# praveer13/zest

Hardware: AMD Instinct MI355X
Metric: aggregate pull GB/s + P2P ratio, Llama-3.1-70B at 1/2/4/8 MI355X peers (higher is better)
Workload: dtype bf16

## Files before the change

csrc/gpu/compress.hip:

```cpp
#include <hip/hip_runtime.h>

#include <cstdint>
#include <cstdlib>

#include "zgpu.h"

namespace {

constexpr int kWave = 64;
constexpr int kWavesPerBlock = 4;
constexpr int kTabLog = 12;
constexpr uint32_t kTab = 1u << kTabLog;

__device__ __forceinline__ uint32_t lane_id() { return threadIdx.x & (kWave - 1); }

__device__ __forceinline__ uint32_t load_u32(const uint8_t* p) {
  const uintptr_t a = reinterpret_cast<uintptr_t>(p);
  const uint32_t k = uint32_t(a & 3);
  const uint32_t* w = reinterpret_cast<const uint32_t*>(a & ~uintptr_t(3));
  const uint32_t w0 = w[0];
  return k == 0 ? w0 : __builtin_amdgcn_alignbyte(w[1], w0, k);
}

__device__ __forceinline__ uint32_t put_len(uint8_t* o, uint32_t op, uint32_t r, uint32_t lane) {
  const uint32_t nff = r / 255;
  for (uint32_t i = lane; i < nff; i += kWave) o[op + i] = 0xFF;
  if (lane == 0) o[op + nff] = uint8_t(r - 255 * nff);
  return op + nff + 1;
}

__device__ __forceinline__ uint32_t emit(uint8_t* o, uint32_t op, const uint8_t* in, uint32_t lit0, uint32_t L,
                                         uint32_t off, uint32_t ml, uint32_t lane) {
  const uint32_t M = ml ? ml - 4 : 0;
  if (lane == 0) o[op] = uint8_t(((L < 15 ? L : 15) << 4) | (ml ? (M < 15 ? M : 15) : 0));
  ++op;
  if (L >= 15) op = put_len(o, op, L - 15, lane);
  for (uint32_t i = lane; i < L; i += kWave) o[op + i] = in[lit0 + i];
  op += L;
  if (ml) {
    if (lane == 0) {
      o[op] = uint8_t(off & 0xFF);
      o[op + 1] = uint8_t(off >> 8);
    }
    op += 2;
    if (M >= 15) op = put_len(o, op, M - 15, lane);
  }
  return op;
}

__global__ void __launch_bounds__(256) k_bg4_split(const uint8_t* __restrict__ data, const uint64_t* __restrict__ offs,
                                                   const uint32_t* __restrict__ lens, int n, uint8_t* __restrict__ out,
                                                   uint64_t slot) {
  const int c = __builtin_amdgcn_readfirstlane(int(blockIdx.x * kWavesPerBlock + (threadIdx.x >> 6)));
  if (c >= n) return;
  const uint32_t lane = lane_id(), len = lens[c];
  const uint8_t* s = data + offs[c];
  uint8_t* d = out + uint64_t(c) * slot;
  const uint32_t q = len >> 2, r = len & 3;
  const uint32_t g1 = q + (r > 0), g2 = g1 + q + (r > 1), g3 = g2 + q + (r > 2);
  for (uint32_t i = lane; i < len; i += kWave) {
    const uint32_t g = i & 3, j = i >> 2;
    const uint32_t base = g == 0 ? 0u : g == 1 ? g1 : g == 2 ? g2 : g3;
    d[base + j] = s[i];
  }
}

__global__ void __launch_bounds__(256) k_lz4_compress_v1(const uint8_t* __restrict__ data, const uint64_t* __restrict__ offs,
                                                      const uint32_t* __restrict__ lens, int n, uint64_t in_slot,
                                                      uint8_t* __restrict__ out, uint64_t out_slot,
                                                      uint32_t* __restrict__ out_len, uint32_t hc64, uint32_t hc256) {
  __shared__ unsigned long long tabs[kWavesPerBlock][kTab];
  const int wave = __builtin_amdgcn_readfirstlane(int(threadIdx.x >> 6));
  const int c = __builtin_amdgcn_readfirstlane(int(blockIdx.x * kWavesPerBlock + wave));
  if (c >= n) return;
  const uint32_t lane = lane_id();
  unsigned long long* tab = tabs[wave];
  for (uint32_t i = lane; i < kTab; i += kWave) tab[i] = 0;
  __builtin_amdgcn_wave_barrier();
  const uint32_t len = lens[c];
  const uint8_t* in = in_slot ? data + uint64_t(c) * in_slot : data + offs[c];
  uint8_t* o = out + uint64_t(c) * out_slot;
  uint32_t op = 11, ip = 0, anchor = 0;
  const uint32_t mend = len > 5 ? len - 5 : 0;
  while (ip + 12 <= len) {
    const uint32_t p = ip + lane;
    const bool ok = p + 12 <= len;
    const uint32_t v = ok ? load_u32(in + p) : 0;
    const uint32_t h = (v * 2654435761u) >> (32 - kTabLog);
    const unsigned long long e = ok ? tab[h] : 0ull;
    uint32_t cand = uint32_t(e >> 32) - 1;
    bool hit = ok && e != 0 && uint32_t(e) == v && cand < p && p - cand <= 65535u;
    uint32_t near = 0;
    for (int d = 32; d >= 1; --d) {
      const uint32_t u = __shfl_up(v, d, kWave);
      if (lane >= uint32_t(d) && u == v) near = d;
    }
    if (ok && near) {
      cand = p - near;
      hit = true;
    }
    const unsigned long long mask = __ballot(hit);
    const uint32_t passed = mask ? uint32_t(__builtin_ctzll(mask)) + 1 : uint32_t(kWave);
    __builtin_amdgcn_wave_barrier();
    if (ok && lane < passed) atomicMax(&tab[h], (static_cast<unsigned long long>(p + 1) << 32) | v);
    if (!mask) {
      ip += kWave;
      continue;
    }
    const int j = __builtin_ctzll(mask);
    uint32_t mp = ip + uint32_t(j);
    uint32_t mc = uint32_t(__builtin_amdgcn_readlane(int(cand), j));
    while (true) {
      const uint32_t room = (mp - anchor) < mc ? (mp - anchor) : mc;
      if (room == 0) break;
      const uint32_t k = lane + 1;
      const bool eq = k <= room && in[mp - k] == in[mc - k];
      const unsigned long long ne = __ballot(!eq);
      const uint32_t b = ne ? uint32_t(__builtin_ctzll(ne)) : uint32_t(kWave);
      mp -= b;
      mc -= b;
      if (b < uint32_t(kWave)) break;
    }
    const uint32_t maxlen = mend - mp;
    uint32_t ml = 4 + (ip + uint32_t(j) - mp);
    while (ml < maxlen) {
      const uint32_t k = ml + lane;
      const bool eq = k < maxlen && in[mc + k] == in[mp + k];
      const unsigned long long ne = __ballot(!eq);
      if (ne) {
        ml += uint32_t(__builtin_ctzll(ne));
        break;
      }
      ml += kWave;
    }
    if (ml > maxlen) ml = maxlen;
    op = emit(o, op, in, anchor, mp - anchor, mp - mc, ml, lane);
    ip = mp + ml;
    anchor = ip;
  }
  op = emit(o, op, in, anchor, len - anchor, 0, 0, lane);
  const uint32_t total = op + 4;
  if (total >= len) {
    if (lane == 0) out_len[c] = 0;
    return;
  }
  if (lane == 0) {
    const uint32_t bs = op - 11;
    const bool small = len <= 65536;
    const uint8_t hdr[11] = {0x04, 0x22, 0x4D, 0x18, 0x60, uint8_t(small ? 0x40 : 0x50),
                             uint8_t(small ? hc64 : hc256), uint8_t(bs), uint8_t(bs >> 8), uint8_t(bs >> 16),
                             uint8_t(bs >> 24)};
    for (int i = 0; i < 11; ++i) o[i] = hdr[i];
    for (int i = 0; i < 4; ++i) o[op + i] = 0;
    out_len[c] = total;
  }
}

constexpr uint32_t kTagBits = 14;
constexpr uint32_t kTagMask = (1u << kTagBits) - 1;
constexpr uint32_t kRing = 4096;
constexpr uint32_t kRingMask = kRing - 1;
constexpr uint32_t kFlush = 2048;
constexpr uint32_t kHdr = 11;

struct Staged {
  uint8_t* ring;
  uint8_t* g;
  uint32_t flushed;
};

__device__ __forceinline__ void ring_write(Staged& o, uint32_t end, uint32_t lane) {
  __builtin_amdgcn_wave_barrier();
  for (uint32_t pos = o.flushed + lane; pos < end; pos += kWave)
    if (pos >= kHdr) o.g[pos] = o.ring[pos & kRingMask];
  __builtin_amdgcn_wave_barrier();
}

__device__ __forceinline__ void maybe_flush(Staged& o, uint32_t op, uint32_t lane) {
  while (op - o.flushed >= kFlush) {
    ring_write(o, o.flushed + kFlush, lane);
    o.flushed += kFlush;
  }
}

__device__ __forceinline__ uint32_t put_len_s(Staged& o, uint32_t op, uint32_t r, uint32_t lane) {
  const uint32_t nff = r / 255;
  for (uint32_t i = lane; i < nff; i += kWave) o.ring[(op + i) & kRingMask] = 0xFF;
  if (lane == 0) o.ring[(op + nff) & kRingMask] = uint8_t(r - 255 * nff);
  return op + nff + 1;
}

__device__ __forceinline__ uint32_t emit_s(Staged& o, uint32_t op, const uint8_t* in, uint32_t lit0, uint32_t L,
                                           uint32_t off, uint32_t ml, uint32_t lane) {
  const uint32_t M = ml ? ml - 4 : 0;
  maybe_flush(o, op, lane);
  if (lane == 0) o.ring[op & kRingMask] = uint8_t(((L < 15 ? L : 15) << 4) | (ml ? (M < 15 ? M : 15) : 0));
  ++op;
  if (L >= 15) op = put_len_s(o, op, L - 15, lane);
  for (uint32_t b = 0; b < L; b += 1024) {
    maybe_flush(o, op + b, lane);
    const uint32_t n = L - b < 1024 ? L - b : 1024;
    for (uint32_t i = lane; i < n; i += kWave) o.ring[(op + b + i) & kRingMask] = in[lit0 + b + i];
  }
  op += L;
  if (ml) {
    maybe_flush(o, op, lane);
    if (lane == 0) {
      o.ring[op & kRingMask] = uint8_t(off & 0xFF);
      o.ring[(op + 1) & kRingMask] = uint8_t(off >> 8);
    }
    op += 2;
    if (M >= 15) op = put_len_s(o, op, M - 15, lane);
  }
  return op;
}

__global__ void __launch_bounds__(256) k_lz4_compress(const uint8_t* __restrict__ data, const uint64_t* __restrict__ offs,
                                                      const uint32_t* __restrict__ lens, int n, uint64_t in_slot,
                                                      uint8_t* __restrict__ out, uint64_t out_slot,
                                                      uint32_t* __restrict__ out_len, uint32_t hc64, uint32_t hc256) {
  __shared__ uint32_t tabs[kWavesPerBlock][kTab];
  __shared__ uint8_t rings[kWavesPerBlock][kRing];
  const int wave = __builtin_amdgcn_readfirstlane(int(threadIdx.x >> 6));
  const int c = __builtin_amdgcn_readfirstlane(int(blockIdx.x * kWavesPerBlock + wave));
  if (c >= n) return;
  const uint32_t lane = lane_id();
  uint32_t* tab = tabs[wave];
  for (uint32_t i = lane; i < kTab; i += kWave) tab[i] = 0;
  __builtin_amdgcn_wave_barrier();
  const uint32_t len = lens[c];
  const uint8_t* in = in_slot ? data + uint64_t(c) * in_slot : data + offs[c];
  Staged o{rings[wave], out + uint64_t(c) * out_slot, 0};
  uint32_t op = kHdr, ip = 0, anchor = 0;
  const uint32_t mend = len > 5 ? len - 5 : 0;
  while (ip + 12 <= len) {
    const uint32_t p = ip + lane;
    const bool ok = p + 12 <= len;
    const uint32_t v = ok ? load_u32(in + p) : 0;
    const uint32_t hv = v * 2654435761u;
    const uint32_t h = hv >> (32 - kTabLog);
    const uint32_t tag = hv & kTagMask;
    const uint32_t e = ok ? tab[h] : 0u;
    uint32_t cand = (e >> kTagBits) - 1;
    bool hit = ok && e != 0 && (e & kTagMask) == tag && cand < p && p - cand <= 65535u;
    if (hit) hit = load_u32(in + cand) == v;
    uint32_t near = 0;
    for (int d = 32; d >= 1; --d) {
      const uint32_t u = __shfl_up(v, d, kWave);
      if (lane >= uint32_t(d) && u == v) near = d;
    }
    if (ok && near) {
      cand = p - near;
      hit = true;
    }
    const unsigned long long mask = __ballot(hit);
    const uint32_t passed = mask ? uint32_t(__builtin_ctzll(mask)) + 1 : uint32_t(kWave);
    __builtin_amdgcn_wave_barrier();
    if (ok && lane < passed) atomicMax(&tab[h], ((p + 1) << kTagBits) | tag);
    if (!mask) {
      ip += kWave;
      continue;
    }
    const int j = __builtin_ctzll(mask);
    uint32_t mp = ip + uint32_t(j);
    uint32_t mc = uint32_t(__builtin_amdgcn_readlane(int(cand), j));
    while (true) {
      const uint32_t room = (mp - anchor) < mc ? (mp - anchor) : mc;
      if (room == 0) break;
      const uint32_t k = lane + 1;
      const bool eq = k <= room && in[mp - k] == in[mc - k];
      const unsigned long long ne = __ballot(!eq);
      const uint32_t b = ne ? uint32_t(__builtin_ctzll(ne)) : uint32_t(kWave);
      mp -= b;
      mc -= b;
      if (b < uint32_t(kWave)) break;
    }
    const uint32_t maxlen = mend - mp;
    uint32_t ml = 4 + (ip + uint32_t(j) - mp);
    while (ml < maxlen) {
      const uint32_t k = ml + lane;
      const bool eq = k < maxlen && in[mc + k] == in[mp + k];
      const unsigned long long ne = __ballot(!eq);
      if (ne) {
        ml += uint32_t(__builtin_ctzll(ne));
        break;
      }
      ml += kWave;
    }
    if (ml > maxlen) ml = maxlen;
    op = emit_s(o, op, in, anchor, mp - anchor, mp - mc, ml, lane);
    ip = mp + ml;
    anchor = ip;
  }
  op = emit_s(o, op, in, anchor, len - anchor, 0, 0, lane);
  const uint32_t total = op + 4;
  if (total >= len) {
    if (lane == 0) out_len[c] = 0;
    return;
  }
  maybe_flush(o, op, lane);
  if (lane < 4) o.ring[(op + lane) & kRingMask] = 0;
  ring_write(o, total, lane);
  if (lane == 0) {
    const uint32_t bs = op - kHdr;
    const bool small = len <= 65536;
    const uint8_t hdr[kHdr] = {0x04, 0x22, 0x4D, 0x18, 0x60, uint8_t(small ? 0x40 : 0x50),
                               uint8_t(small ? hc64 : hc256), uint8_t(bs), uint8_t(bs >> 8), uint8_t(bs >> 16),
                               uint8_t(bs >> 24)};
    for (uint32_t i = 0; i < kHdr; ++i) o.g[i] = hdr[i];
    out_len[c] = total;
  }
}

bool compress_v1() {
  const char* e = getenv("ZG_COMPRESS");
  return e && e[0] == 'v' && e[1] == '1';
}

__global__ void __launch_bounds__(256) k_pack_frames(const uint64_t* __restrict__ src, const uint32_t* __restrict__ clen,
                                                     const uint32_t* __restrict__ ulen, const uint8_t* __restrict__ scheme,
                                                     const uint64_t* __restrict__ out_off, int n, uint8_t* __restrict__ out) {
  const int c = __builtin_amdgcn_readfirstlane(int(blockIdx.x * kWavesPerBlock + (threadIdx.x >> 6)));
  if (c >= n) return;
  const uint32_t lane = lane_id(), cl = clen[c], ul = ulen[c];
  uint8_t* d = out + out_off[c];
  if (lane < 8) {
    const uint32_t b = lane == 0 ? 0u : lane < 4 ? (cl >> (8 * (lane - 1))) & 0xFF
                                  : lane == 4 ? scheme[c] : (ul >> (8 * (lane - 5))) & 0xFF;
    d[lane] = uint8_t(b);
  }
  const uint8_t* s = reinterpret_cast<const uint8_t*>(src[c]);
  for (uint32_t i = lane; i < cl; i += kWave) d[8 + i] = s[i];
}

}

extern "C" {

hipError_t zg_compress_chunks(const uint8_t* data, const uint64_t* offs, const uint32_t* lens, int n, int bg4,
                              uint8_t* scratch, uint64_t in_slot, uint8_t* out, uint64_t out_slot, uint32_t* out_len,
                              uint32_t hc64, uint32_t hc256, hipStream_t stream) {
  if (n <= 0) return hipSuccess;
  const dim3 grid((n + kWavesPerBlock - 1) / kWavesPerBlock);
  auto* kern = compress_v1() ? k_lz4_compress_v1 : k_lz4_compress;
  if (bg4) {
    hipLaunchKernelGGL(k_bg4_split, grid, dim3(256), 0, stream, data, offs, lens, n, scratch, in_slot);
    hipLaunchKernelGGL(kern, grid, dim3(256), 0, stream, scratch, offs, lens, n, in_slot, out, out_slot, out_len,
                       hc64, hc256);
  } else {
    hipLaunchKernelGGL(kern, grid, dim3(256), 0, stream, data, offs, lens, n, uint64_t(0), out, out_slot, out_len,
                       hc64, hc256);
  }
  return hipGetLastError();
}

hipError_t zg_pack_frames(const uint64_t* src, const uint32_t* clen, const uint32_t* ulen, const uint8_t* scheme,
                          const uint64_t* out_off, int n, uint8_t* out, hipStream_t stream) {
  if (n <= 0) return hipSuccess;
  hipLaunchKernelGGL(k_pack_frames, dim3((n + kWavesPerBlock - 1) / kWavesPerBlock), dim3(256), 0, stream, src, clen,
                     ulen, scheme, out_off, n, out);
  return hipGetLastError();
}

}
```

Before: 62.46.

## Stage LZ4 input in a register window read via ds_bpermute

The compressor keeps a sliding window of input in wave registers (four rows of 256 bytes plus a prefetch row) and reads hash words, candidate verification bytes, short match extensions and literals through ds_bpermute instead of scattered global byte loads. Candidate checking becomes a loop that compares a 64-byte span around each hit, which gives the backward and forward extension for free inside that span. It is meant to cut global memory latency in the match-finding loop. In exchange it adds many bpermute operations per step, more registers per lane, and a more complex control flow, which may lower occupancy.

```diff
diff --git a/csrc/gpu/compress.hip b/csrc/gpu/compress.hip
--- a/csrc/gpu/compress.hip
+++ b/csrc/gpu/compress.hip
@@ -190,17 +190,112 @@
   return op + nff + 1;
 }
 
-__device__ __forceinline__ uint32_t emit_s(Staged& o, uint32_t op, const uint8_t* in, uint32_t lit0, uint32_t L,
-                                           uint32_t off, uint32_t ml, uint32_t lane) {
+constexpr uint32_t kRow = 4 * kWave;
+constexpr uint32_t kWinRows = 4;
+constexpr uint32_t kWin = kRow * kWinRows;
+constexpr uint32_t kSpanBack = 16;
+constexpr uint32_t kSpanFwd = kWave - kSpanBack - 4;
+
+struct Window {
+  uint32_t w0, w1, w2, w3, nxt;
+  const uint32_t* base;
+  uint32_t a0, endq;
+  int32_t wq;
+};
+
+__device__ __forceinline__ uint32_t win_load_row(const Window& W, int32_t q0, uint32_t lane) {
+  const uint32_t q = uint32_t(q0) + 4 * lane;
+  return q < W.endq ? W.base[q >> 2] : 0u;
+}
+
+__device__ __forceinline__ void win_load_all(Window& W, int32_t wq, uint32_t lane) {
+  W.wq = wq;
+  W.w0 = win_load_row(W, wq, lane);
+  W.w1 = win_load_row(W, wq + int32_t(kRow), lane);
+  W.w2 = win_load_row(W, wq + int32_t(2 * kRow), lane);
+  W.w3 = win_load_row(W, wq + int32_t(3 * kRow), lane);
+  W.nxt = win_load_row(W, wq + int32_t(kWin), lane);
+}
+
+__device__ __forceinline__ void win_advance(Window& W, uint32_t ip, uint32_t lane) {
+  const int32_t ipq = int32_t(ip + W.a0);
+  if (ipq < W.wq + int32_t(2 * kRow)) return;
+  if (ipq < W.wq + int32_t(3 * kRow)) {
+    W.w0 = W.w1;
+    W.w1 = W.w2;
+    W.w2 = W.w3;
+    W.w3 = W.nxt;
+    W.wq += int32_t(kRow);
+    W.nxt = win_load_row(W, W.wq + int32_t(kWin), lane);
+  } else {
+    win_load_all(W, (ipq & ~int32_t(kRow - 1)) - int32_t(kRow), lane);
+  }
+}
+
+__device__ __forceinline__ bool win_holds(const Window& W, uint32_t lo, uint32_t hi) {
+  return int32_t(lo + W.a0) >= W.wq && int32_t(hi + W.a0) <= W.wq + int32_t(kWin);
+}
+
+__device__ __forceinline__ uint32_t bperm(uint32_t src_lane, uint32_t x) {
+  return uint32_t(__builtin_amdgcn_ds_bpermute(int(src_lane << 2), int(x)));
+}
+
+__device__ __forceinline__ uint32_t win_byte(const Window& W, uint32_t p) {
+  const uint32_t o = (p + W.a0 - uint32_t(W.wq)) & (kWin - 1);
+  const uint32_t l = (o >> 2) & (kWave - 1), r = o >> 8;
+  const uint32_t t0 = bperm(l, W.w0), t1 = bperm(l, W.w1), t2 = bperm(l, W.w2), t3 = bperm(l, W.w3);
+  const uint32_t d = r == 0 ? t0 : r == 1 ? t1 : r == 2 ? t2 : t3;
+  return (d >> (8 * (o & 3))) & 0xFFu;
+}
+
+__device__ __forceinline__ uint32_t win_u32(const Window& W, uint32_t ip, uint32_t lane) {
+  const uint32_t o = ip + W.a0 - uint32_t(W.wq) + lane;
+  const uint32_t d0 = o >> 2, d1 = d0 + 1;
+  const uint32_t a1 = bperm(d0 & (kWave - 1), W.w1), a2 = bperm(d0 & (kWave - 1), W.w2);
+  const uint32_t b1 = bperm(d1 & (kWave - 1), W.w1), b2 = bperm(d1 & (kWave - 1), W.w2);
+  const uint32_t lo = d0 < 2 * kWave ? a1 : a2, hi = d1 < 2 * kWave ? b1 : b2;
+  return __builtin_amdgcn_alignbyte(hi, lo, o & 3);
+}
+
+__device__ __forceinline__ unsigned long long span_eq(const Window& W, const uint8_t* in, uint32_t len, uint32_t mp0,
+                                                      uint32_t mc0, uint32_t lane) {
+  const uint32_t mpos = mp0 - kSpanBack + lane, cpos = mc0 - kSpanBack + lane;
+  const uint32_t clo = mc0 > kSpanBack ? mc0 - kSpanBack : 0u;
+  const uint32_t chi = mc0 + kSpanFwd + 4 < len ? mc0 + kSpanFwd + 4 : len;
+  const uint32_t mb = win_byte(W, mpos);
+  uint32_t cb;
+  if (win_holds(W, clo, chi)) {
+    cb = win_byte(W, cpos);
+  } else {
+    cb = cpos < len ? uint32_t(in[cpos]) : 0u;
+  }
+  return __ballot(mpos < len && cpos < len && mb == cb);
+}
+
+__device__ __forceinline__ uint32_t emit_s(Staged& o, uint32_t op, const uint8_t* in, const Window& W, uint32_t ip,
+                                           uint32_t vw, uint32_t lit0, uint32_t L, uint32_t off, uint32_t ml,
+                                           uint32_t lane) {
   const uint32_t M = ml ? ml - 4 : 0;
   maybe_flush(o, op, lane);
   if (lane == 0) o.ring[op & kRingMask] = uint8_t(((L < 15 ? L : 15) << 4) | (ml ? (M < 15 ? M : 15) : 0));
   ++op;
   if (L >= 15) op = put_len_s(o, op, L - 15, lane);
-  for (uint32_t b = 0; b < L; b += 1024) {
-    maybe_flush(o, op + b, lane);
-    const uint32_t n = L - b < 1024 ? L - b : 1024;
-    for (uint32_t i = lane; i < n; i += kWave) o.ring[(op + b + i) & kRingMask] = in[lit0 + b + i];
+  if (L && lit0 >= ip && lit0 + L <= ip + kWave) {
+    maybe_flush(o, op, lane);
+    const uint32_t b = bperm((lit0 - ip + lane) & (kWave - 1), vw);
+    if (lane < L) o.ring[(op + lane) & kRingMask] = uint8_t(b);
+  } else if (L && win_holds(W, lit0, lit0 + L)) {
+    maybe_flush(o, op, lane);
+    for (uint32_t i = 0; i < L; i += kWave) {
+      const uint32_t b = win_byte(W, lit0 + i + lane);
+      if (i + lane < L) o.ring[(op + i + lane) & kRingMask] = uint8_t(b);
+    }
+  } else {
+    for (uint32_t b = 0; b < L; b += 1024) {
+      maybe_flush(o, op + b, lane);
+      const uint32_t n = L - b < 1024 ? L - b : 1024;
+      for (uint32_t i = lane; i < n; i += kWave) o.ring[(op + b + i) & kRingMask] = in[lit0 + b + i];
+    }
   }
   op += L;
   if (ml) {
@@ -231,19 +326,25 @@
   const uint32_t len = lens[c];
   const uint8_t* in = in_slot ? data + uint64_t(c) * in_slot : data + offs[c];
   Staged o{rings[wave], out + uint64_t(c) * out_slot, 0};
+  Window W;
+  W.a0 = uint32_t(reinterpret_cast<uintptr_t>(in) & 3);
+  W.base = reinterpret_cast<const uint32_t*>(in - W.a0);
+  W.endq = W.a0 + len;
+  win_load_all(W, -int32_t(kRow), lane);
   uint32_t op = kHdr, ip = 0, anchor = 0;
   const uint32_t mend = len > 5 ? len - 5 : 0;
   while (ip + 12 <= len) {
+    win_advance(W, ip, lane);
     const uint32_t p = ip + lane;
     const bool ok = p + 12 <= len;
-    const uint32_t v = ok ? load_u32(in + p) : 0;
+    const uint32_t vw = win_u32(W, ip, lane);
+    const uint32_t v = ok ? vw : 0;
     const uint32_t hv = v * 2654435761u;
     const uint32_t h = hv >> (32 - kTabLog);
     const uint32_t tag = hv & kTagMask;
     const uint32_t e = ok ? tab[h] : 0u;
     uint32_t cand = (e >> kTagBits) - 1;
-    bool hit = ok && e != 0 && (e & kTagMask) == tag && cand < p && p - cand <= 65535u;
-    if (hit) hit = load_u32(in + cand) == v;
+    bool maybe = ok && e != 0 && (e & kTagMask) == tag && cand < p && p - cand <= 65535u;
     uint32_t near = 0;
     for (int d = 32; d >= 1; --d) {
       const uint32_t u = __shfl_up(v, d, kWave);
@@ -251,48 +352,73 @@
     }
     if (ok && near) {
       cand = p - near;
-      hit = true;
-    }
-    const unsigned long long mask = __ballot(hit);
-    const uint32_t passed = mask ? uint32_t(__builtin_ctzll(mask)) + 1 : uint32_t(kWave);
+      maybe = true;
+    }
+    unsigned long long todo = __ballot(maybe), eq = 0;
+    uint32_t j = 0, mc = 0;
+    bool found = false;
+    while (todo) {
+      j = uint32_t(__builtin_ctzll(todo));
+      mc = uint32_t(__builtin_amdgcn_readlane(int(cand), int(j)));
+      eq = span_eq(W, in, len, ip + j, mc, lane);
+      if (((eq >> kSpanBack) & 0xF) == 0xF) {
+        found = true;
+        break;
+      }
+      todo &= todo - 1;
+    }
+    const uint32_t passed = found ? j + 1 : uint32_t(kWave);
     __builtin_amdgcn_wave_barrier();
     if (ok && lane < passed) atomicMax(&tab[h], ((p + 1) << kTagBits) | tag);
-    if (!mask) {
+    if (!found) {
       ip += kWave;
       continue;
     }
-    const int j = __builtin_ctzll(mask);
-    uint32_t mp = ip + uint32_t(j);
-    uint32_t mc = uint32_t(__builtin_amdgcn_readlane(int(cand), j));
-    while (true) {
+    uint32_t mp = ip + j;
+    {
       const uint32_t room = (mp - anchor) < mc ? (mp - anchor) : mc;
-      if (room == 0) break;
-      const uint32_t k = lane + 1;
-      const bool eq = k <= room && in[mp - k] == in[mc - k];
-      const unsigned long long ne = __ballot(!eq);
-      const uint32_t b = ne ? uint32_t(__builtin_ctzll(ne)) : uint32_t(kWave);
+      const uint32_t ne = ~uint32_t(eq) & ((1u << kSpanBack) - 1);
+      uint32_t b = ne ? uint32_t(__builtin_clz(ne)) - (32 - kSpanBack) : kSpanBack;
+      if (b > room) b = room;
       mp -= b;
       mc -= b;
-      if (b < uint32_t(kWave)) break;
+      while (b == kSpanBack) {
+        const uint32_t room2 = (mp - anchor) < mc ? (mp - anchor) : mc;
+        if (room2 == 0) break;
+        const uint32_t k = lane + 1;
+        const bool same = k <= room2 && in[mp - k] == in[mc - k];
+        const unsigned long long diff = __ballot(!same);
+        const uint32_t s = diff ? uint32_t(__builtin_ctzll(diff)) : uint32_t(kWave);
+        mp -= s;
+        mc -= s;
+        if (s < uint32_t(kWave)) break;
+      }
     }
     const uint32_t maxlen = mend - mp;
-    uint32_t ml = 4 + (ip + uint32_t(j) - mp);
-    while (ml < maxlen) {
-      const uint32_t k = ml + lane;
-      const bool eq = k < maxlen && in[mc + k] == in[mp + k];
-      const unsigned long long ne = __ballot(!eq);
-      if (ne) {
-        ml += uint32_t(__builtin_ctzll(ne));
-        break;
+    uint32_t ml = 4 + (ip + j - mp);
+    {
+      const unsigned long long ne = ~eq >> (kSpanBack + 4);
+      const uint32_t f = ne ? uint32_t(__builtin_ctzll(ne)) : kSpanFwd;
+      ml += f;
+      if (f == kSpanFwd) {
+        while (ml < maxlen) {
+          const uint32_t k = ml + lane;
+          const bool same = k < maxlen && in[mc + k] == in[mp + k];
+          const unsigned long long diff = __ballot(!same);
+          if (diff) {
+            ml += uint32_t(__builtin_ctzll(diff));
+            break;
+          }
+          ml += kWave;
+        }
       }
-      ml += kWave;
     }
     if (ml > maxlen) ml = maxlen;
-    op = emit_s(o, op, in, anchor, mp - anchor, mp - mc, ml, lane);
+    op = emit_s(o, op, in, W, ip, vw, anchor, mp - anchor, mp - mc, ml, lane);
     ip = mp + ml;
     anchor = ip;
   }
-  op = emit_s(o, op, in, anchor, len - anchor, 0, 0, lane);
+  op = emit_s(o, op, in, W, ~0u, 0u, anchor, len - anchor, 0, 0, lane);
   const uint32_t total = op + 4;
   if (total >= len) {
     if (lane == 0) out_len[c] = 0;
diff --git a/profiles/compress_window/step0.py b/profiles/compress_window/step0.py
--- /dev/null
+++ b/profiles/compress_window/step0.py
@@ -0,0 +1,53 @@
+#!/usr/bin/env python3
+import sys
+from pathlib import Path
+
+import numpy as np
+
+ROOT = Path(__file__).resolve().parents[2]
+sys.path.insert(0, str(ROOT))
+sys.path.insert(0, str(ROOT / "tests"))
+
+import lz4_compress_model as M
+from zest_amd.synthetic import _host_fill
+
+
+def hist(vals, edges):
+    vals = np.asarray(vals)
+    out = []
+    for lo, hi in zip(edges[:-1], edges[1:]):
+        out.append((f"{lo}..{hi - 1}", int(((vals >= lo) & (vals < hi)).sum())))
+    return out
+
+
+def main(nchunks=8, size=65536):
+    buf = np.empty(nchunks * size, dtype=np.uint8)
+    _host_fill(buf, 7, 1)
+    tot = dict.fromkeys(M.STAT_KEYS, 0)
+    offs, mls, lits = [], [], []
+    for c in range(nchunks):
+        src = M.bg4_split_np(buf[c * size:(c + 1) * size].tobytes())
+        st = {}
+        frame = M.compress_model(src, st)
+        for k in M.STAT_KEYS:
+            tot[k] += st[k]
+        _, seqs = M.parse_frame(frame, size)
+        for nl, off, ml in seqs:
+            lits.append(nl)
+            if ml:
+                offs.append(off)
+                mls.append(ml)
+    n = nchunks
+    print(f"chunks {n} x {size}: per chunk windows {tot['windows'] / n:.0f}, sequences {tot['sequences'] / n:.0f}, "
+          f"near hits {tot['near_hits'] / n:.0f}, table hits {tot['far_hits'] / n:.0f}, "
+          f"tag rejects {tot['tag_reject'] / n:.1f}, backward extensions {tot['back_ext'] / n:.0f}, "
+          f"frame {tot['frame_len'] / n:.0f} B")
+    for name, vals, edges in (("offset", offs, (1, 33, 64, 256, 1024, 4096, 16384, 65536)),
+                              ("match length", mls, (4, 5, 6, 8, 12, 20, 68, 132, 1 << 17)),
+                              ("literals", lits, (0, 1, 2, 4, 8, 16, 64, 256, 1024, 1 << 17))):
+        total = len(vals)
+        print(name + ": " + ", ".join(f"{r}: {k} ({100 * k / total:.1f} %)" for r, k in hist(vals, edges)))
+
+
+if __name__ == "__main__":
+    main()
```

After: 62.41. About the same (-0.1%).
